# tartarughina/S-BLAS

Hardware: AMD Instinct MI355X
Metric: SpMM GFLOP/s (2*nnz*N/t), CSR x dense N=64, fp64 (higher is better)
Workload: dtype f64; 1 GPU; SpMM method-1 (dense-B column partition), nd24k-like synthetic (M=K=72000, 399 nnz/row, band +-2000, seed 211), nnz=28728000, N=64 columns per GPU, alpha=beta=1, B = srand(211)/rand() as the reference's DenseMatrix, inputs resident in HBM; step = B->row-major staging + row-panel SpMM; rows=72000, cols=72000, nnz=28728000, n_cols_per_gpu=64, parallelism=method1-colblock x1

## Files before the change

include/sblas_hip.h:

```cpp
#ifndef SBLAS_HIP_H
#define SBLAS_HIP_H

#include <stddef.h>
#include <stdint.h>

#ifdef __cplusplus
extern "C" {
#endif

#define SBLAS_OK 0
#define SBLAS_E_INVALID 1
#define SBLAS_E_HIP 2
#define SBLAS_E_WORKSPACE 3
#define SBLAS_E_RCCL 4
#define SBLAS_E_IO 5
#define SBLAS_E_NOGPU 6

int sblas_hip_version(void);
const char *sblas_hip_error_string(int code);
int sblas_hip_device_count(void);

size_t sblas_hip_spmm_csr_f64_i32_workspace(int64_t rows, int64_t cols, int64_t nnz, int64_t n);

int sblas_hip_spmm_csr_f64_i32(int dev, void *stream,
// ... 272 lines not shown
    SBLAS_SPMM_RULE_FOUR_ROWS_WAVES,
    SBLAS_SPMM_RULE_FOUR_ROWS_VOTED,
    SBLAS_SPMM_RULE_MERGE,
    SBLAS_SPMM_RULE_DPP_GROUPS,
    SBLAS_SPMM_RULE_DPP_PAD,
    SBLAS_SPMM_RULE_DPP_LONG,
    SBLAS_SPMM_RULE_NARROW,
    SBLAS_SPMM_RULE_ROWS8,
    SBLAS_SPMM_RULE_INTERLEAVE,
    SBLAS_SPMM_RULE_SKIP,
    SBLAS_SPMM_RULE_SPLIT_GROUPS,
    SBLAS_SPMM_RULE_FIELDS
};
int64_t sblas_spmm_rule_describe(int64_t rows, int64_t cols, int64_t nnz, int64_t ldbt, int64_t n, int64_t ncu,
                                 int caller_staged, const int64_t *plan, int64_t *out, int64_t max_out);

int sblas_host_fill_rand0to1(double *dst, int64_t count, unsigned seed);

int sblas_mm_read_info(const char *path, int32_t *rows, int32_t *cols, int32_t *nnz,
                       int32_t *is_symmetric);
int sblas_mm_read_csr(const char *path, int32_t *rowptr, int32_t *colidx, double *val);

#ifdef __cplusplus
}
#endif
#endif
```

s-blas_amd/csrc/kernels.h:

```cpp
#pragma once
#include <hip/hip_runtime.h>
#include <stdint.h>
#include <vector>
#include "../../include/sblas_hip.h"

namespace sblas {

constexpr int MAX_REPLICAS = 16;
struct ReplicaPtrs {
    double *p[MAX_REPLICAS];
};

enum {
    SPMM_VARIANT_AUTO = 0,
    SPMM_VARIANT_DIRECT_DPP = 1,
    SPMM_VARIANT_DIRECT_ROWS = 2,
    SPMM_VARIANT_LANES = 3,
    SPMM_VARIANT_DIRECT_MERGE = 4,
    SPMM_VARIANT_MFMA = 5,
    SPMM_VARIANT_NO_MFMA = 6,
};
constexpr int SPMM_MIN_PANEL_ROWS = 32;

enum { TAIL_NONFINITE = 0,
// ... 24 lines not shown
__device__ __forceinline__ float c_fma(float a, float b, float c) { return fmaf(a, b, c); }
template <int W, typename T, typename At, typename Keep>
__device__ __forceinline__ void store_rows_c(T *__restrict__ C, int64_t ldc, int64_t row0, int64_t col0, int prows, int nrows,
                                             int ncols, int nthreads, T alpha, T beta, At at, Keep keep)
{
    for (int idx = threadIdx.x; idx < W * prows; idx += nthreads) {
        const int j = idx % W, r = idx / W;
        if (r < nrows && j < ncols && keep(r)) {
            T *dst = C + (row0 + r) * ldc + (col0 + j);
            const T sres = alpha * at(r, j);
            *dst = (beta == T(0)) ? sres : c_fma(beta, *dst, sres);
        }
    }
}

__device__ __forceinline__ int xcd_contiguous_panel(int b, int npanels)
{
    const int xcd = b & 7, idx = b >> 3;
    const int q = npanels >> 3, r = npanels & 7;
    const int base = (xcd < r) ? xcd * (q + 1) : r * (q + 1) + (xcd - r) * q;
    return base + idx;
}

struct Options {
    int spmm_variant = SPMM_VARIANT_AUTO;
    char spmv_variant[16] = {0};
    bool tier16 = true, tier32 = true;
    unsigned long long max_bt_bytes = 0xffffffffull;
    int direct_lds = -1;
    int direct_map = -1;
    int stage_range = -1;
    int direct_merge = 1;
    double rows8_min_avg = 256.0;
    float window_density = 0.42f;
    int panel_rows = 0, panel_groups = 0;
    int lanes_copies = 1;
    size_t mfma_lds_floor = 0;
    bool one_half = false;
    int rowlen_bar = 0;
    int mfma_batch64 = 2;
    int mfma_batch128 = 2;
    int dpp_long = DPP_LONG;
    bool lanes32_one_lane = false;
    int rows_waves = 0;
    bool validate = false;
    float mfma_min_fill = -1.0f;
};
const Options &options();
void options_reload();
int compute_units();
// ... 69 lines not shown
SpmmStep spmm_step(int rows, int cols, int64_t nnz, int64_t ldbt, const PlanView *pv, const SpmmStep &prev = SpmmStep(),
                   bool caller_staged = false);
struct ClassifyArgs {
    int max_row_len;
    float min_density, min_rowlen, mfma_min_fill;
    int merge_probe;
};
ClassifyArgs classify_args(int panel_rows, int64_t ldbt);
int range_parts(int64_t nnz);

enum { TILED_NONE = 0, TILED_WINDOW6 = 1 , TILED_LANES = 2  };
struct SpmmStage2 {
    int tiled = TILED_NONE;
    int g = 0;
    int nh = 0, grid_y = 0;
    int nc = 0, cp = 0, lpe = 0;
    bool mfma = false;
    int mfma_batch = 0;
    size_t mfma_lds_floor = 0;
    bool four_rows = false;
    int rows_waves = 0, voted = 0;
    bool merge = false;
    int dpp = 0;
    size_t dpp_pad = 0;
    int dpp_long = 0;
    int narrow = 0;
    bool rows8 = false;
    int interleave = -1;
    bool skip = false;
    int split_groups = 0;
};
SpmmStage2 spmm_stage2(const SpmmStep &st, int rows, int cols, int64_t nnz, int n);
hipError_t launch_stage(hipStream_t s, const SpmmStep &st, int rows, int64_t cols, int64_t nnz, const int *rowptr,
                        const int *colidx, int64_t n, const double *B, int64_t ldb, double *Bt, bool row_b);
hipError_t launch_spmm_rowpanel(hipStream_t s, const SpmmStep &st, int rows, int cols, int64_t nnz, const int *rowptr,
                                const int *colidx, const double *val, const double *Bt, int n, double alpha, double beta,
                                double *C, int64_t ldc, bool row_c);
hipError_t plan_build(hipStream_t s, const SpmmStep &st, int rows, int cols, int64_t nnz, const int *rowptr, const int *colidx,
                      PlanView *pv, std::vector<int> *cls_out = nullptr);
hipError_t launch_dense_to_rowmajor(hipStream_t s, int64_t cols, int64_t n, const double *B, int64_t ldb,
                                    double *Bt, int64_t ldbt, bool row_b);
hipError_t launch_scale(hipStream_t s, int64_t rows, int64_t n, double beta, double *C, int64_t ldc, bool row_c);
hipError_t validate_csr(hipStream_t s, int64_t rows, int64_t cols, int64_t nnz, const int *rowptr, const int *colidx, int *bad);
hipError_t panel_stats(unsigned long long out[4], bool reset);
hipError_t launch_spmv(hipStream_t s, int rows, int cols, int64_t nnz, const int *rowptr, const int *colidx,
                       const double *val, const double *x, double alpha, double beta, double *y);
int spmv_kind(double avg, int family = -1);
// ... 42 lines not shown
```

s-blas_amd/csrc/kernels.hip:

```cpp
#include <hip/hip_runtime.h>
#include <atomic>
#include <stdint.h>
#include <algorithm>
#include <type_traits>
#include <mutex>
#include <vector>
#include "kernels.h"

namespace sblas {

constexpr int WAVE = 64;

__device__ __forceinline__ int wave_uniform(int v) { return __builtin_amdgcn_readfirstlane(v); }

__device__ __forceinline__ double readlane_f64(double v, int src_lane)
{
    int lo = __double2loint(v), hi = __double2hiint(v);
    lo = __builtin_amdgcn_readlane(lo, src_lane);
    hi = __builtin_amdgcn_readlane(hi, src_lane);
    return __hiloint2double(hi, lo);
}

constexpr int STAGE_K = 32;
template <bool RB>
// ... 207 lines not shown
        for (; k < cnt; ++k) {
            const int c = __builtin_amdgcn_readlane(cj, k);
            const double a = readlane_f64(vj, k);
            acc = fma(a, (Bt + (size_t)((unsigned)c * ld32))[lane_off], acc);
        }
    }
    return acc;
}
#ifndef SBLAS_W2_ROWS
#define SBLAS_W2_ROWS 152
#endif
constexpr int W2_ROWS = SBLAS_W2_ROWS;
constexpr int W2_LROWS = W2_ROWS / 4;
static_assert(W2_ROWS % 8 == 0, "tile rows");
constexpr int W2_TILE = W2_ROWS * 64;
constexpr size_t W2_LDS_BYTES = (2 * (size_t)W2_TILE + 64) * sizeof(double) + 64 * sizeof(int);

constexpr int MFMA_BITMAP_WORDS = 1024;
__device__ __forceinline__ void classify_panel(int p, int rows, int cols, int npanels, int panel_rows,
                                               const int *__restrict__ rowptr, const int *__restrict__ colidx,
                                               ClassifyArgs a, int *__restrict__ tail, int2 *__restrict__ info,
                                               int *__restrict__ cls, int epoch, unsigned *__restrict__ bitmap)
{
    const int max_row_len = a.max_row_len, merge_probe = a.merge_probe;
    const float min_density = a.min_density, min_rowlen = a.min_rowlen, mfma_min_fill = a.mfma_min_fill;
    const int lane = threadIdx.x & 63;
    if (p >= npanels) return;
    int first = 0x7fffffff, last = -1, len = 0, mlen = 0;
    for (int rr = lane; rr < panel_rows; rr += WAVE) {
        const int row = p * panel_rows + rr;
        if (row < rows) {
// ... 426 lines not shown
template <int N> __device__ __forceinline__ void vm_wait6()
{
    static_assert(N == 8 || N == 12, "counts of the sixth-generation tile loop");
    if (N == 12) asm volatile("s_waitcnt vmcnt(12)" ::: "memory");
    else asm volatile("s_waitcnt vmcnt(8)" ::: "memory");
}

template <int G, int NH, bool RC>
__global__ __launch_bounds__(1024) void spmm_window6_kernel(
    int rows, int cols, int npanels, const int *__restrict__ rowptr, const int *__restrict__ colidx,
    const double *__restrict__ val, const double *__restrict__ Bt, int64_t ldbt, int n, double alpha, double beta,
    double *__restrict__ C, int64_t ldc, const int *__restrict__ tail, const int2 *__restrict__ info,
    const int *__restrict__ cls, int panel_rows, int nnz)
{
    constexpr int RW = 4 * G, RMAX = 16 * RW;
    static_assert(G == 2 || G == 3, "two or three groups per wave (the counted vmcnt waits are 4 G)");
    static_assert(NH == 1 || NH == 2, "one or two 64-column halves per workgroup");
    static_assert(64 * (RMAX + 1) <= 2 * W2_TILE, "C tile must fit in the (dead) B tile buffers");
    extern __shared__ __attribute__((aligned(16))) double smem[];
    double *zero_row = smem + 2 * W2_TILE;
    int *sm_i = reinterpret_cast<int *>(smem + 2 * W2_TILE + 64);

    const int panel = xcd_contiguous_panel(blockIdx.x, npanels);
    if (!owns_window(tail, cls, panel)) return;
    const int2 span = info[panel];

    const int tid = threadIdx.x;
    const int lane = tid & 63;
    const int wave = wave_uniform(tid >> 6);
    const int row0 = panel * panel_rows;
    const int col0 = blockIdx.y * (64 * NH);
    const unsigned ld32 = (unsigned)ldbt;
    const int t_lo = span.x / W2_ROWS, t_hi = span.y / W2_ROWS;
    const bool loader = wave >= 12;
    const bool active = !loader && wave * RW < panel_rows;

    if (tid < 64) zero_row[tid] = 0.0;
    if (tid == 0) sm_i[0] = 0;

    double acc[NH][G][4];
#pragma unroll
    for (int h = 0; h < NH; ++h)
#pragma unroll
        for (int g = 0; g < G; ++g)
#pragma unroll
            for (int j = 0; j < 4; ++j) acc[h][g][j] = 0.0;

    const unsigned ldb8 = ld32 * 8u;
    const unsigned piece_off = (unsigned)(col0 + ((lane & 31) << 1)) * 8u;
    const unsigned pair_off = (unsigned)(lane >> 5) * ldb8 + piece_off;
    const char *bt_bytes = reinterpret_cast<const char *>(Bt);
    int dummy = 0;
    auto dma_part = [&](int t, int h, int buf) {
        const int lw = wave - 12;
        const int r0 = t * W2_ROWS + lw * W2_LROWS;
        const unsigned lds0 = (unsigned)wave_uniform((int)((unsigned)(uintptr_t)(smem + buf * W2_TILE) + (unsigned)lw * (unsigned)(W2_LROWS * 512)));
        const unsigned hoff = (unsigned)h * 512u;
        if (r0 + W2_LROWS - 1 <= cols) {
            const char *p = bt_bytes + (size_t)((unsigned)r0 * ldb8) + hoff;
#pragma unroll
            for (int i = 0; i < W2_LROWS / 2; ++i) dma_rows_scalar(lds0 + i * 1024u, pair_off, p + (size_t)(2u * i) * ldb8);
        } else {
#pragma unroll
            for (int i = 0; i < W2_LROWS / 2; ++i) {
                const unsigned brow = (unsigned)min(r0 + 2 * i + (lane >> 5), cols);
                dma_rows_vector(lds0 + i * 1024u, bt_bytes + (size_t)(brow * ldb8 + piece_off + hoff));
            }
        }
    };

    if (loader) dma_part(t_lo, 0, 0);

    const int k = lane & 15, q = lane >> 4;
    const int wrow = min(row0 + wave * RW, rows);
    const int wstart = wave_uniform(rowptr[wrow]);
    const sblas_rsrc_t rc = make_rsrc(colidx + wstart, 4u, (unsigned)(nnz - wstart));
    const sblas_rsrc_t rv = make_rsrc(val + wstart, 8u, (unsigned)(nnz - wstart));
    int cur[G], end[G];
#pragma unroll
    for (int g = 0; g < G; ++g) {
        const int rr = wave * RW + 4 * g + q;
        const int row = row0 + rr;
        cur[g] = end[g] = 0;
        if (rr < panel_rows && row < rows) {
            cur[g] = rowptr[row] - wstart;
            end[g] = rowptr[row + 1] - wstart;
        }
    }
    unsigned long long viol = 0ull;
    int wca[G], wcb[G];
    double wva[G], wvb[G];
    unsigned s_coA[G], s_coB[G];
    double s_gvA[G], s_gvB[G];
    int s_take[G], s_mx[G];
    bool replay[G];
#pragma unroll
    for (int g = 0; g < G; ++g) {
        s_coA[g] = s_coB[g] = 0u;
        s_gvA[g] = s_gvB[g] = 0.0;
        s_take[g] = s_mx[g] = 0;
        replay[g] = false;
    }
#pragma unroll
    for (int g = 0; g < G; ++g) window_issue6(rc, rv, cur[g] + k, wca[g], wva[g], wcb[g], wvb[g]);
    asm volatile("s_waitcnt vmcnt(0)" ::: "memory");
    __syncthreads();
    int step = 0;
    for (int t = t_lo; t <= t_hi; ++t) {
        const int tile_lo = t * W2_ROWS;
        auto half = [&](auto hc) {
            constexpr int h = decltype(hc)::value;
            const int cbuf = step & 1;
            if (loader) {
                if (h + 1 < NH) dma_part(t, h + 1, cbuf ^ 1);
                else if (t < t_hi) dma_part(t + 1, 0, cbuf ^ 1);
            }
            const unsigned tile_base = (unsigned)(uintptr_t)(smem + cbuf * W2_TILE);
            const unsigned lb = tile_base + (unsigned)k * 16u;
            const unsigned zero_rel = (unsigned)(uintptr_t)zero_row - tile_base;
            auto visit = [&](auto gc) {
                constexpr int g = decltype(gc)::value;
                if (h == 0) window_wait6<NH == 1 ? 4 * (G - 1) : 4 * (G - 1 - g)>(wca[g], wva[g], wcb[g], wvb[g]);
                else if (replay[g]) window_wait6<0>(wca[g], wva[g], wcb[g], wvb[g]);
                double &q0 = acc[h][g][0], &q1 = acc[h][g][1], &q2 = acc[h][g][2], &q3 = acc[h][g][3];
                int lc = cur[g];
                bool full = h == 0 || replay[g];
                for (;;) {
                    unsigned coA, coB;
                    double gvA, gvB;
                    int take, mx;
// ... 60 lines not shown
            ++step;
        };
        half(std::integral_constant<int, 0>{});
        if constexpr (NH > 1) half(std::integral_constant<int, 1>{});
    }
#pragma unroll
    for (int g = 0; g < G; ++g) window_wait6<0>(wca[g], wva[g], wcb[g], wvb[g]);
    int bad = viol != 0ull ? 1 : 0;
#pragma unroll
    for (int g = 0; g < G; ++g)
        if (__builtin_amdgcn_ballot_w64(cur[g] < end[g]) != 0ull) bad = 1;
    if (bad && lane == 0) atomicOr(&sm_i[0], 1);
    __syncthreads();
    const bool fell_back = sm_i[0] != 0;
    if (tid == 0 && blockIdx.y == 0) atomicAdd(&g_panel_stats[fell_back ? 2 : 0], 1ull);

    double *ctile = smem;
    const int nrows = min(panel_rows, rows - row0);
#pragma unroll
    for (int h = 0; h < NH; ++h) {
        const int colh = col0 + 64 * h;
        if (fell_back) {
            const unsigned lane_off = (unsigned)(colh + lane);
#pragma unroll
            for (int g = 0; g < G; ++g)
#pragma unroll
                for (int j = 0; j < 4; ++j) {
                    const int rr = wave * RW + 4 * g + j;
                    const int row = row0 + rr;
                    int a = 0, b = 0;
// ... 6 lines not shown
        }
        if (h > 0) __syncthreads();
#pragma unroll
        for (int g = 0; g < G; ++g) {
            if (fell_back) {
#pragma unroll
                for (int j = 0; j < 4; ++j) ctile[lane * (RMAX + 1) + wave * RW + 4 * g + j] = acc[h][g][j];
            } else {
                const int rr = wave * RW + 4 * g + q;
                ctile[(2 * k) * (RMAX + 1) + rr] = acc[h][g][0];
                ctile[(2 * k + 1) * (RMAX + 1) + rr] = acc[h][g][1];
                ctile[(32 + 2 * k) * (RMAX + 1) + rr] = acc[h][g][2];
                ctile[(33 + 2 * k) * (RMAX + 1) + rr] = acc[h][g][3];
            }
        }
        __syncthreads();
        const int ncols = min(64, n - colh);
        if constexpr (RC)
            store_rows_c<64>(C, ldc, row0, colh, panel_rows, nrows, ncols, 1024, alpha, beta,
                             [&](int r, int j) { return ctile[j * (RMAX + 1) + r]; }, [](int) { return true; });
        else
        for (int idx = tid; idx < 64 * panel_rows; idx += 1024) {
            const int r = idx % panel_rows, j = idx / panel_rows;
            if (r < nrows && j < ncols) {
                double *dst = C + (int64_t)(colh + j) * ldc + (row0 + r);
                const double sres = alpha * ctile[j * (RMAX + 1) + r];
                *dst = (beta == 0.0) ? sres : fma(beta, *dst, sres);
            }
        }
    }
}

constexpr int WL_TR = 256;
template <int NC, int CP> struct WlGeom {
    static constexpr int P = NC / 2;
    static constexpr unsigned ROWB = NC * 8;
    static constexpr unsigned ROW = CP * ROWB;
    static constexpr int SHIFT = ROW == 64 ? 6 : ROW == 128 ? 7 : 8;
    static constexpr unsigned TILE = WL_TR * ROW;
    static constexpr size_t LDS_BYTES = 2 * (size_t)TILE + 512 + 64;
    static constexpr int LPR = CP * P;
    static constexpr int RPI = 64 / LPR;
    static_assert(ROW == 64 || ROW == 128 || ROW == 256, "copies x row bytes");
    static_assert(CP * P <= 16, "a lane group has sixteen lanes");
};
// ... 386 lines not shown
    static_assert(GROUPS == 1 || GROUPS == 2 || GROUPS == 4, "lane groups of 64, 32 or 16 lanes");
    constexpr int TILE_COLS = 128 / GROUPS;
    constexpr int GLANES = 64 / GROUPS;
    __shared__ double ctile[TILE_COLS][WIDE_PANEL + 1];
    if (cls != nullptr && nothing_direct(tail, epoch)) return;
    if (GROUPS == 1 && cls != nullptr && (tail[TAIL_MERGE_EPOCH] == epoch || tail[TAIL_ROWS_EPOCH] == epoch)) return;
    const int lane = threadIdx.x & 63;
    const int wave = wave_uniform(threadIdx.x >> 6);
    if (interleave < 0) {
        interleave = 0;
        if (cls != nullptr) {
            const int band = tail[TAIL_BAND];
            interleave = (long long)band * (TILE_COLS * 8) > (16ll << 20);
        }
    }
    const int row0 = (interleave ? (int)blockIdx.x : xcd_contiguous_panel(blockIdx.x, npanels)) * WIDE_PANEL;
    const int col0 = blockIdx.y * TILE_COLS;
    const int row = row0 + wave;
    bool mine = row < rows;
    if (cls && mine) {
        mine = owns_direct(tail, cls, row / info_panel_rows);
        if (mine && lane == 0 && blockIdx.y == 0 && row % info_panel_rows == 0) atomicAdd(&g_panel_stats[1], 1ull);
    }
    if (SKIP && mine) mine = !is_split_row(split_bits, row);
    const int sub = lane & 15;
    const int half = lane / GLANES;
    const unsigned ldb8 = (unsigned)ldbt * 8u;
    const unsigned lb = (unsigned)(col0 * 8) + (unsigned)(lane % GLANES) * 16u;
    const unsigned zero_off = (unsigned)cols * ldb8;
    const char *__restrict__ bt_bytes = reinterpret_cast<const char *>(Bt);

    double acc0 = 0.0, acc1 = 0.0;
    auto sweep = [&](int p0, int p1) { dpp_sweep<GROUPS>(colidx, val, bt_bytes, ldb8, lb, zero_off, lane, sub, half, p0, p1, acc0, acc1); };
    __shared__ int long_wave[WIDE_PANEL];
    __shared__ int n_long;
    if (threadIdx.x == 0) n_long = 0;
    __syncthreads();
    int rp0 = 0, rp1 = 0;
    if (mine) {
        rp0 = wave_uniform(rowptr[row]);
        rp1 = wave_uniform(rowptr[row + 1]);
    }
    const bool is_long = mine && rp1 - rp0 >= long_min;
    if (is_long && lane == 0) long_wave[atomicAdd(&n_long, 1)] = wave;
    if (mine && !is_long) sweep(rp0, rp1);
    if (GROUPS == 4) {
        acc0 += __shfl_xor(acc0, 16, WAVE);
        acc1 += __shfl_xor(acc1, 16, WAVE);
// ... 42 lines not shown
        }
    }
    const int nrows = min(WIDE_PANEL, rows - row0);
    const int ncols = min(TILE_COLS, n - col0);
    if constexpr (RC)
        store_rows_c<TILE_COLS>(C, ldc, row0, col0, WIDE_PANEL, nrows, ncols, WIDE_WAVES * 64, alpha, beta,
                                [&](int r, int j) { return ctile[j][r]; }, [&](int r) { return row_mine[r] != 0; });
    else
    for (int idx = threadIdx.x; idx < TILE_COLS * WIDE_PANEL; idx += WIDE_WAVES * 64) {
        const int r = idx % WIDE_PANEL, j = idx / WIDE_PANEL;
        if (r < nrows && j < ncols && row_mine[r]) {
            double *dst = C + (int64_t)(col0 + j) * ldc + (row0 + r);
            const double sres = alpha * ctile[j][r];
            *dst = (beta == 0.0) ? sres : fma(beta, *dst, sres);
        }
    }
}

constexpr int MR = 3;
constexpr int MERGE_WAVES = 8;
constexpr int MERGE_PANEL = MERGE_WAVES * MR;
template <int NR>
__device__ __forceinline__ void merged_sweeps(int cj, const double (&vj)[NR], int cnt, double (&acc)[NR][2], int sub,
                                              unsigned ldb8, unsigned lb, unsigned zero_off,
                                              const char *__restrict__ bt_bytes)
{
    for (int g0 = 0; g0 < cnt; g0 += 16) {
        const int e = g0 + sub;
        const int src = e << 2;
        const bool on = e < cnt;
// ... 815 lines not shown
    const SpmmStage2 d = spmm_stage2(st, rows, cols, nnz, n);
    const int64_t ldbt = st.ldbt;
    const PlanView *pv = st.pv;
    const Tail t = pv ? tail_at(pv->tail, rows) : tail_of(Bt, cols, ldbt, rows);
    const bool classified = st.verdicts != VERDICTS_NONE;
    const int *cls = classified ? t.cls : nullptr;
    const int info_rows = st.info_rows, np = st.npanels, epoch = st.epoch;
    const unsigned *skip = d.skip ? pv->split_bits : nullptr;
    bool missing = false;
    if (classified && !pv) launch_verdicts(s, st, rows, cols, rowptr, colidx, t, st.verdicts == VERDICTS_SEPARATE);

    if (classified) {
        KernelEvents *kev = kernel_events_slot();
        if (kev) (void)hipEventRecord(kev->a, s);
        if (d.tiled == TILED_WINDOW6) {
            const dim3 wgrid((unsigned)np, (unsigned)d.grid_y);
#define SBLAS_W6_CASE(GG, NH)                                                                                          \
    case GG * 10 + NH:                                                                                                \
        raise_dynamic_lds((const void *)spmm_window6_kernel<GG, NH, RC>, W2_LDS_BYTES);                               \
        hipLaunchKernelGGL((spmm_window6_kernel<GG, NH, RC>), wgrid, dim3(1024), W2_LDS_BYTES, s, rows, cols, np, rowptr,   \
                           colidx, val, Bt, ldbt, n, alpha, beta, C, ldc, t.hdr, t.info, t.cls, info_rows, (int)nnz); \
        break;
            switch (d.g * 10 + d.nh) {
                SBLAS_W6_CASE(2, 1) SBLAS_W6_CASE(2, 2) SBLAS_W6_CASE(3, 1)
            default: missing = true;
            }
#undef SBLAS_W6_CASE
        } else if (d.tiled == TILED_LANES) {
#define SBLAS_LANES_CASE(NC, CP, GG, LPE)                                                                              \
    case ((NC * 10 + CP) * 10 + GG) * 10 + LPE:                                                                       \
        raise_dynamic_lds((const void *)spmm_lanes_kernel<NC, CP, GG, LPE, RC>, WlGeom<NC, CP>::LDS_BYTES);           \
// ... 36 lines not shown
            SBLAS_ROWS_CASE(4) SBLAS_ROWS_CASE(8) SBLAS_ROWS_CASE(16)
        default: missing = true;
        }
#undef SBLAS_ROWS_CASE
    }
    if (d.merge) {
        const int mp = (rows + MERGE_PANEL - 1) / MERGE_PANEL;
        const size_t lds = (size_t)128 * (MERGE_PANEL + 1) * sizeof(double);
        raise_dynamic_lds((const void *)spmm_direct_merge_kernel<RC>, lds);
        hipLaunchKernelGGL(spmm_direct_merge_kernel<RC>, dim3((unsigned)mp, (unsigned)(ldbt / 128)), dim3(MERGE_WAVES * 64), lds,
                           s, rows, cols, mp, rowptr, colidx, val, Bt, ldbt, n, alpha, beta, C, ldc, t.hdr, cls, info_rows,
                           d.interleave, epoch);
    }
    if (d.dpp) {
        const int wide_panels = (rows + WIDE_PANEL - 1) / WIDE_PANEL;
        const dim3 grid((unsigned)wide_panels, d.dpp == 1 ? (unsigned)(ldbt / 128) : 1u);
#define SBLAS_DPP_CASE(GR)                                                                                             \
    case GR:                                                                                                          \
        SBLAS_DIRECT_GO(spmm_direct_dpp_kernel, (GR, RC), grid, dim3(WIDE_WAVES * 64), d.dpp_pad, rows, cols, wide_panels,  \
                        rowptr, colidx, val, Bt, ldbt, n, alpha, beta, C, ldc, t.hdr, cls, info_rows, d.interleave, epoch,   \
                        d.dpp_long);                                                                                  \
        break;
        switch (d.dpp) {
            SBLAS_DPP_CASE(1) SBLAS_DPP_CASE(2) SBLAS_DPP_CASE(4)
        default: missing = true;
        }
#undef SBLAS_DPP_CASE
    }
    if (d.narrow) {
        const unsigned panels = (unsigned)((rows + PANEL_ROWS - 1) / PANEL_ROWS);
#define SBLAS_NARROW_CASE(NC)                                                                                          \
// ... 104 lines not shown
```

s-blas_amd/csrc/spmm_rule.cpp:

```cpp
#include <stdint.h>
#include <stdio.h>
#include <stdlib.h>
#include <string.h>
#include <algorithm>
#include <atomic>
#include <mutex>
#include "../../include/sblas_hip.h"
#include "kernels.h"

namespace sblas {

static Options g_options;
static std::atomic<bool> g_options_loaded{false};
static std::mutex g_options_mu;
static void options_parse(Options &o)
{
    o = Options{};
    const char *e;
    if ((e = getenv("SBLAS_SPMM_VARIANT")) && *e) {
        if (!strcmp(e, "dpp")) o.spmm_variant = SPMM_VARIANT_DIRECT_DPP;
        else if (!strcmp(e, "rows")) o.spmm_variant = SPMM_VARIANT_DIRECT_ROWS;
        else if (!strcmp(e, "lanes")) o.spmm_variant = SPMM_VARIANT_LANES;
        else if (!strcmp(e, "merge")) o.spmm_variant = SPMM_VARIANT_DIRECT_MERGE;
        else if (!strcmp(e, "mfma")) o.spmm_variant = SPMM_VARIANT_MFMA;
// ... 5 lines not shown
    if ((e = getenv("SBLAS_SPMM_MIN_LDBT")) && *e) o.tier16 = o.tier32 = atoi(e) < 64;
    if ((e = getenv("SBLAS_SPMM_MAX_BT_BYTES")) && *e) {
        const unsigned long long v = strtoull(e, nullptr, 10);
        if (v >= 4096 && v < 0xffffffffull) o.max_bt_bytes = v;
    }
    if ((e = getenv("SBLAS_DIRECT_LDS")) && *e) o.direct_lds = atoi(e);
    if ((e = getenv("SBLAS_DIRECT_MERGE")) && *e) o.direct_merge = atoi(e);
    if ((e = getenv("SBLAS_STAGE_RANGE")) && *e) o.stage_range = atoi(e);
    if ((e = getenv("SBLAS_DIRECT_MAP")) && *e) o.direct_map = !strcmp(e, "interleave") ? 1 : !strcmp(e, "contiguous") ? 0 : -1;
    if ((e = getenv("SBLAS_ROWS8_MIN_AVG")) && *e) o.rows8_min_avg = atof(e);
    if ((e = getenv("SBLAS_WINDOW_DENSITY")) && *e) o.window_density = (float)atof(e);
    if ((e = getenv("SBLAS_SPMM_PANEL_ROWS")) && *e) {
        o.panel_rows = atoi(e);
        o.panel_groups = strchr(e, ',') ? atoi(strchr(e, ',') + 1) : 0;
    }
    if ((e = getenv("SBLAS_MFMA_MIN_FILL")) && *e) o.mfma_min_fill = (float)atof(e);
    if ((e = getenv("SBLAS_VALIDATE")) && *e) o.validate = atoi(e) != 0;
    if ((e = getenv("SBLAS_TUNE")) && *e) {
        char buf[96];
        strncpy(buf, e, sizeof buf - 1);
        buf[sizeof buf - 1] = 0;
        for (char *c = buf; *c; ++c)
            if (*c == ':') *c = ',';
        int a = 0, b = 0, c = 0, d = 0;
        sscanf(buf, "%d,%d,%d,%d", &a, &b, &c, &d);
        if (a == 2 || a == 4) o.lanes_copies = a;
        if (a > 0 && a <= 160 * 1024) o.mfma_lds_floor = (size_t)a;
        o.one_half = b == 1;
        if (b > 1) o.rowlen_bar = b;
        if (b == 3 || b == 4) o.mfma_batch64 = b;
// ... 153 lines not shown
        st.npanels = (int)(((int64_t)rows + st.info_rows - 1) / st.info_rows);
    }
    again = classify && range && prev.staging == STAGE_RANGE && prev.verdicts != VERDICTS_NONE && prev.ldbt == ldbt;
    st.verdicts = !classify ? VERDICTS_NONE : again ? VERDICTS_EARLIER : caller_staged ? VERDICTS_SEPARATE : VERDICTS_STAGING;
    return st;
}

SpmmStep spmm_step(int rows, int cols, int64_t nnz, int64_t ldbt, const PlanView *pv, const SpmmStep &prev, bool caller_staged)
{
    bool again = false;
    SpmmStep st = step_rule(rows, cols, nnz, ldbt, pv, prev, caller_staged, 0, again);
    st.epoch = pv ? pv->epoch : again ? prev.epoch : next_epoch();
    return st;
}

SpmmStage2 spmm_stage2(const SpmmStep &st, int rows, int cols, int64_t nnz, int n)
{
    SpmmStage2 d;
    const Options &opt = options();
    const int variant = opt.spmm_variant;
    const int64_t ldbt = st.ldbt;
    const PlanView *pv = st.pv;
    const double avg_row = rows > 0 ? (double)nnz / (double)rows : 0.0;
    const bool classified = st.verdicts != VERDICTS_NONE;
    const bool need_window = !pv || pv->n_window + pv->n_mfma_w > 0;
    const bool need_mfma = !pv || pv->n_mfma_w + pv->n_mfma_d > 0;
    const bool need_direct = !pv || pv->n_direct + pv->n_mfma_d > 0;
    d.g = st.groups;
    d.interleave = opt.direct_map;
    d.dpp_long = opt.dpp_long;
    d.skip = pv && pv->n_split > 0;
    d.split_groups = ldbt >= 128 ? 1 : ldbt == 64 ? 2 : 4;
    d.rows_waves = opt.rows_waves ? opt.rows_waves : avg_row < 8.0 ? 4 : 16;
    if (ldbt >= 64) {
        if (classified) {
            const bool two_halves = ldbt >= 128 && !opt.one_half;
            if (need_window) {
                d.tiled = TILED_WINDOW6;
                d.g = st.groups == 3 ? 3 : 2;
                d.nh = d.g == 2 && two_halves ? 2 : 1;
                d.grid_y = (int)(ldbt / (two_halves ? 128 : 64));
            }
            d.mfma = need_mfma && mfma_min_fill(variant, st.info_rows, ldbt) <= 1.0f;
            d.mfma_batch = ldbt == 64 ? opt.mfma_batch64 : opt.mfma_batch128;
            d.mfma_lds_floor = opt.mfma_lds_floor;
        }
        d.dpp_pad = opt.direct_lds >= 0 ? (size_t)opt.direct_lds : (ldbt == 64 ? 0 : 90000);
        if (!need_direct) {
        } else if (n > 32 && (variant == SPMM_VARIANT_DIRECT_ROWS ||
                              (variant != SPMM_VARIANT_DIRECT_DPP && avg_row < (ldbt == 64 ? 56.0 : 32.0)))) {
            d.four_rows = true;
        } else if (ldbt == 64) {
            d.dpp = n <= 32 ? 4 : 2;
        } else {
            d.merge = pv ? pv->merge : variant == SPMM_VARIANT_DIRECT_MERGE || (classified && opt.direct_merge);
            d.dpp = (pv ? !pv->merge && !pv->four_rows : variant != SPMM_VARIANT_DIRECT_MERGE) ? 1 : 0;
            d.four_rows = pv ? pv->four_rows : classified && variant != SPMM_VARIANT_DIRECT_MERGE;
// ... 43 lines not shown
    if (plan) {
        for (int k = 0; k < SBLAS_SPMM_RULE_PLAN_FIELDS; ++k)
            if (plan[k] < 0) return -1;
        if (plan[SBLAS_SPMM_RULE_PLAN_PANEL_ROWS] < 1 || plan[SBLAS_SPMM_RULE_PLAN_PANEL_ROWS] > INT32_MAX ||
            plan[SBLAS_SPMM_RULE_PLAN_GROUPS] > INT32_MAX || caller_staged)
            return -1;
        pv.n_window = (long)plan[SBLAS_SPMM_RULE_PLAN_N_WINDOW], pv.n_direct = (long)plan[SBLAS_SPMM_RULE_PLAN_N_DIRECT];
        pv.n_mfma_w = (long)plan[SBLAS_SPMM_RULE_PLAN_N_MFMA_W], pv.n_mfma_d = (long)plan[SBLAS_SPMM_RULE_PLAN_N_MFMA_D];
        pv.merge = plan[SBLAS_SPMM_RULE_PLAN_MERGE] != 0, pv.four_rows = plan[SBLAS_SPMM_RULE_PLAN_FOUR_ROWS] != 0;
        pv.n_split = plan[SBLAS_SPMM_RULE_PLAN_N_SPLIT];
        pv.info_rows = (int)plan[SBLAS_SPMM_RULE_PLAN_PANEL_ROWS], pv.groups = (int)plan[SBLAS_SPMM_RULE_PLAN_GROUPS];
    }
    bool again = false;
    const sblas::SpmmStep st = sblas::step_rule((int)rows, (int)cols, nnz, ldbt, plan ? &pv : nullptr, sblas::SpmmStep(),
                                                caller_staged != 0, (int)ncu, again);
    const sblas::SpmmStage2 d = sblas::spmm_stage2(st, (int)rows, (int)cols, nnz, (int)n);
    int64_t f[SBLAS_SPMM_RULE_FIELDS] = {0};
    f[SBLAS_SPMM_RULE_STAGING] = st.staging, f[SBLAS_SPMM_RULE_VERDICTS] = st.verdicts;
    f[SBLAS_SPMM_RULE_PANEL_ROWS] = st.info_rows, f[SBLAS_SPMM_RULE_GROUPS] = st.groups;
    f[SBLAS_SPMM_RULE_PANELS] = st.npanels, f[SBLAS_SPMM_RULE_PLANNABLE] = st.plannable;
    f[SBLAS_SPMM_RULE_TILED] = d.tiled, f[SBLAS_SPMM_RULE_TILED_G] = d.tiled ? d.g : 0;
    f[SBLAS_SPMM_RULE_W6_NH] = d.nh, f[SBLAS_SPMM_RULE_W6_GRID_Y] = d.grid_y;
    f[SBLAS_SPMM_RULE_LANES_NC] = d.nc, f[SBLAS_SPMM_RULE_LANES_CP] = d.cp, f[SBLAS_SPMM_RULE_LANES_LPE] = d.lpe;
    f[SBLAS_SPMM_RULE_MFMA] = d.mfma;
    f[SBLAS_SPMM_RULE_MFMA_BATCH] = d.mfma ? d.mfma_batch : 0;
    f[SBLAS_SPMM_RULE_MFMA_LDS_FLOOR] = d.mfma ? (int64_t)d.mfma_lds_floor : 0;
    f[SBLAS_SPMM_RULE_FOUR_ROWS] = d.four_rows;
    f[SBLAS_SPMM_RULE_FOUR_ROWS_WAVES] = d.four_rows ? d.rows_waves : 0;
    f[SBLAS_SPMM_RULE_FOUR_ROWS_VOTED] = d.voted;
    f[SBLAS_SPMM_RULE_MERGE] = d.merge;
    f[SBLAS_SPMM_RULE_DPP_GROUPS] = d.dpp;
    f[SBLAS_SPMM_RULE_DPP_PAD] = d.dpp ? (int64_t)d.dpp_pad : 0;
    f[SBLAS_SPMM_RULE_DPP_LONG] = d.dpp ? d.dpp_long : 0;
    f[SBLAS_SPMM_RULE_NARROW] = d.narrow, f[SBLAS_SPMM_RULE_ROWS8] = d.rows8;
    f[SBLAS_SPMM_RULE_INTERLEAVE] = d.interleave;
    f[SBLAS_SPMM_RULE_SKIP] = d.skip, f[SBLAS_SPMM_RULE_SPLIT_GROUPS] = d.skip ? d.split_groups : 0;
    for (int64_t k = 0; out && k < SBLAS_SPMM_RULE_FIELDS && k < max_out; ++k) out[k] = f[k];
    return SBLAS_SPMM_RULE_FIELDS;
}
```

s-blas_amd/python/sblas_amd/__init__.py:

```python
import ctypes as C
import os

import numpy as np

_PKG = os.path.dirname(os.path.abspath(__file__))
_ROOT = os.path.normpath(os.path.join(_PKG, "..", ".."))
LIB_PATH = os.environ.get("SBLAS_LIB_PATH") or os.path.join(_ROOT, "lib", "libsblas_hip.so")

EXPORTS = [
    "sblas_hip_version", "sblas_hip_error_string", "sblas_hip_device_count",
    "sblas_hip_spmm_csr_f64_i32_workspace", "sblas_hip_spmm_csr_f64_i32", "sblas_hip_spmm_ldbt",
    "sblas_hip_dense_to_rowmajor_f64", "sblas_hip_spmm_csr_rowmajorB_f64_i32",
    "sblas_hip_debug_spmm_panel_stats", "sblas_hip_debug_reload_env",
    "sblas_hip_debug_spmm_kernel_events", "sblas_hip_debug_spmm_last_kernel_ms", "sblas_hip_spmv_csr_f64_i32", "sblas_hip_axpby_f64",
    "sblas_hip_comm_get", "sblas_hip_comm_release_all", "sblas_hip_allreduce_sum_f64",
    "sblas_hip_merge_rowblocks_f64", "sblas_hip_merge_rowblocks_local_f64",
    "sblas_find_row_of_nnz", "sblas_partition_nnz", "sblas_partition_dense",
    "sblas_mm_read_info", "sblas_mm_read_csr", "sblas_host_fill_rand0to1",
    "sblas_hip_spmm_csr_workspace", "sblas_hip_spmm_csr", "sblas_hip_spmv_csr", "sblas_hip_axpby",
    "sblas_hip_allreduce_sum", "sblas_hip_merge_rowblocks", "sblas_partition_nnz_i64",
    "sblas_hip_debug_validate_csr_i32",
    "sblas_hip_spmm_plan_create", "sblas_hip_spmm_plan_destroy", "sblas_hip_spmm_plan_info", "sblas_hip_spmm_csr_f64_i32_planned",
    "sblas_hip_spmv_plan_create", "sblas_hip_spmv_plan_destroy", "sblas_hip_spmv_plan_info", "sblas_hip_spmv_csr_f64_i32_planned",
    "sblas_spmv_plan_classify",
    "sblas_hip_spmm_csr_ordered", "sblas_hip_spmm_csr_ordered_f64_i32_planned", "sblas_hip_merge_rowblocks_ordered",
    "sblas_hip_spmm_plan_create_split", "sblas_hip_spmm_plan_split_info", "sblas_spmm_split_classify",
    "sblas_spmm_rule_describe",
    "sblas_hip_csr_transpose_workspace", "sblas_hip_csr_transpose_f64_i32", "sblas_hip_gather_f64",
    "sblas_hip_transpose_plan_create", "sblas_hip_transpose_plan_update_values", "sblas_hip_transpose_plan_info",
    "sblas_hip_transpose_plan_csc", "sblas_hip_transpose_plan_destroy", "sblas_hip_spmv_csr_t_f64_i32_planned",
    "sblas_hip_spmm_csr_t_f64_i32_planned",
    "sblas_hip_coo_to_csr_workspace", "sblas_hip_coo_to_csr_f64_i32", "sblas_hip_coo_plan_create", "sblas_hip_coo_plan_info",
    "sblas_hip_coo_plan_csr", "sblas_hip_coo_plan_assemble", "sblas_hip_coo_plan_destroy",
    "sblas_hip_sddmm_csr_workspace", "sblas_hip_sddmm_csr_f64_i32",
    "sblas_hip_csr_softmax_workspace", "sblas_hip_csr_softmax_f64_i32", "sblas_hip_csr_softmax_backward_f64_i32",
    "sblas_hip_csr_attention_workspace", "sblas_hip_csr_attention_f64_i32", "sblas_hip_csr_attention_backward_f64_i32",
    "sblas_hip_spgemm_limits", "sblas_hip_spgemm_classify", "sblas_hip_spgemm_group_width", "sblas_hip_spgemm_check_nnz",
    "sblas_hip_spgemm_plan_create", "sblas_hip_spgemm_plan_info", "sblas_hip_spgemm_plan_csr", "sblas_hip_spgemm_plan_numeric",
    "sblas_hip_spgemm_plan_destroy",
    "sblas_hip_sptrsv_limits", "sblas_sptrsv_levels", "sblas_sptrsv_schedule",
    "sblas_hip_sptrsv_plan_create", "sblas_hip_sptrsv_plan_info", "sblas_hip_sptrsv_plan_order", "sblas_hip_sptrsv_plan_destroy",
    "sblas_hip_sptrsv_f64_i32_planned", "sblas_hip_sptrsm_f64_i32_planned",
# ... 26 lines not shown
    L.sblas_hip_spmm_csr_f64_i32_workspace.argtypes = [i64, i64, i64, i64]
    L.sblas_hip_spmm_csr_f64_i32.restype = C.c_int
    L.sblas_hip_spmm_csr_f64_i32.argtypes = [C.c_int, vp, i64, i64, i64, vp, vp, vp, vp, i64, i64, f64, f64, vp, i64, vp, sz]
    L.sblas_hip_debug_validate_csr_i32.restype = C.c_int
    L.sblas_hip_debug_validate_csr_i32.argtypes = [C.c_int, vp, i64, i64, i64, vp, vp]
    L.sblas_hip_spmm_plan_create.restype = C.c_int
    L.sblas_hip_spmm_plan_create.argtypes = [C.c_int, vp, i64, i64, i64, vp, vp, i64, C.POINTER(vp)]
    L.sblas_hip_spmm_plan_create_split.restype = C.c_int
    L.sblas_hip_spmm_plan_create_split.argtypes = [C.c_int, vp, i64, i64, i64, vp, vp, i64, i64, i64, C.POINTER(vp)]
    L.sblas_hip_spmm_plan_split_info.restype = C.c_int
    L.sblas_hip_spmm_plan_split_info.argtypes = [vp, C.POINTER(i64)]
    L.sblas_spmm_split_classify.restype = i64
    L.sblas_spmm_split_classify.argtypes = [vp, i64, i64, i64, i64, vp, i64, vp, i64]
    L.sblas_spmm_rule_describe.restype = i64
    L.sblas_spmm_rule_describe.argtypes = [i64, i64, i64, i64, i64, i64, C.c_int, vp, vp, i64]
    L.sblas_hip_spmm_plan_destroy.restype = C.c_int
    L.sblas_hip_spmm_plan_destroy.argtypes = [vp]
    L.sblas_hip_spmm_plan_info.restype = C.c_int
    L.sblas_hip_spmm_plan_info.argtypes = [vp, C.POINTER(i64)]
    L.sblas_hip_spmm_csr_f64_i32_planned.restype = C.c_int
    L.sblas_hip_spmm_csr_f64_i32_planned.argtypes = [vp, C.c_int, vp, i64, i64, i64, vp, vp, vp, vp, i64, i64, f64, f64, vp, i64, vp, sz]
    L.sblas_hip_spmv_plan_create.restype = C.c_int
    L.sblas_hip_spmv_plan_create.argtypes = [C.c_int, vp, i64, i64, i64, vp, vp, C.POINTER(vp)]
    L.sblas_hip_spmv_plan_destroy.restype = C.c_int
    L.sblas_hip_spmv_plan_destroy.argtypes = [vp]
    L.sblas_hip_spmv_plan_info.restype = C.c_int
    L.sblas_hip_spmv_plan_info.argtypes = [vp, C.POINTER(i64)]
    L.sblas_hip_spmv_csr_f64_i32_planned.restype = C.c_int
    L.sblas_hip_spmv_csr_f64_i32_planned.argtypes = [vp, C.c_int, vp, i64, i64, i64, vp, vp, vp, vp, f64, f64, vp]
    L.sblas_spmv_plan_classify.restype = i64
# ... 1495 lines not shown
```

Measured before the change: 15530 GFLOP/s.

## Make window6 and direct-DPP SpMM kernels persistent with next-panel prefetch

The window6 row-panel kernel becomes persistent: its grid is capped near the CU count and each workgroup walks panels in rounds. While it finishes the current panel it prefetches the next panel's row pointers, spans and first B tile into LDS, so the next panel's startup overlaps the current epilogue. The direct-DPP kernel likewise loops over wide panels with a grid capped at four times the CU count. The aim is to cut launch and tail imbalance and hide per-panel startup latency, at the cost of more complex synchronisation, more LDS for the row-pointer records, and the risk of load imbalance from static round-robin assignment.

```diff
diff --git a/include/sblas_hip.h b/include/sblas_hip.h
--- a/include/sblas_hip.h
+++ b/include/sblas_hip.h
@@ -310,6 +310,7 @@
 };
 int64_t sblas_spmm_rule_describe(int64_t rows, int64_t cols, int64_t nnz, int64_t ldbt, int64_t n, int64_t ncu,
                                  int caller_staged, const int64_t *plan, int64_t *out, int64_t max_out);
+int64_t sblas_spmm_walk_describe(int64_t npanels, int64_t grid, int64_t ncu, int64_t *out, int64_t max_out);
 
 int sblas_host_fill_rand0to1(double *dst, int64_t count, unsigned seed);
 
diff --git a/s-blas_amd/csrc/kernels.h b/s-blas_amd/csrc/kernels.h
--- a/s-blas_amd/csrc/kernels.h
+++ b/s-blas_amd/csrc/kernels.h
@@ -62,12 +62,17 @@
     }
 }
 
-__device__ __forceinline__ int xcd_contiguous_panel(int b, int npanels)
+__host__ __device__ __forceinline__ int xcd_contiguous_panel(int b, int npanels)
 {
     const int xcd = b & 7, idx = b >> 3;
     const int q = npanels >> 3, r = npanels & 7;
     const int base = (xcd < r) ? xcd * (q + 1) : r * (q + 1) + (xcd - r) * q;
     return base + idx;
+}
+__host__ __device__ __forceinline__ int walk_panel(int b, int r, int grid, int npanels)
+{
+    const long long v = (long long)b + (long long)r * grid;
+    return v < npanels ? xcd_contiguous_panel((int)v, npanels) : -1;
 }
 
 struct Options {
@@ -82,6 +87,7 @@
     double rows8_min_avg = 256.0;
     float window_density = 0.42f;
     int panel_rows = 0, panel_groups = 0;
+    int w6_grid = 0;
     int lanes_copies = 1;
     size_t mfma_lds_floor = 0;
     bool one_half = false;
@@ -181,6 +187,7 @@
     int tiled = TILED_NONE;
     int g = 0;
     int nh = 0, grid_y = 0;
+    int grid_x = 0;
     int nc = 0, cp = 0, lpe = 0;
     bool mfma = false;
     int mfma_batch = 0;
@@ -194,10 +201,12 @@
     int narrow = 0;
     bool rows8 = false;
     int interleave = -1;
+    int direct_cap = 0;
     bool skip = false;
     int split_groups = 0;
 };
-SpmmStage2 spmm_stage2(const SpmmStep &st, int rows, int cols, int64_t nnz, int n);
+SpmmStage2 spmm_stage2(const SpmmStep &st, int rows, int cols, int64_t nnz, int n, int ncu = 0);
+int w6_grid_x(int npanels, int ncu);
 hipError_t launch_stage(hipStream_t s, const SpmmStep &st, int rows, int64_t cols, int64_t nnz, const int *rowptr,
                         const int *colidx, int64_t n, const double *B, int64_t ldb, double *Bt, bool row_b);
 hipError_t launch_spmm_rowpanel(hipStream_t s, const SpmmStep &st, int rows, int cols, int64_t nnz, const int *rowptr,
diff --git a/s-blas_amd/csrc/kernels.hip b/s-blas_amd/csrc/kernels.hip
--- a/s-blas_amd/csrc/kernels.hip
+++ b/s-blas_amd/csrc/kernels.hip
@@ -245,7 +245,10 @@
 constexpr int W2_LROWS = W2_ROWS / 4;
 static_assert(W2_ROWS % 8 == 0, "tile rows");
 constexpr int W2_TILE = W2_ROWS * 64;
-constexpr size_t W2_LDS_BYTES = (2 * (size_t)W2_TILE + 64) * sizeof(double) + 64 * sizeof(int);
+constexpr int W6_SM_INTS = 256, W6_REC = 8, W6_REC_RP = 12;
+static_assert(W6_REC_RP + 48 * W6_GMAX + 1 <= W6_SM_INTS, "row pointers of the tallest panel");
+constexpr size_t W2_LDS_BYTES = (2 * (size_t)W2_TILE + 64) * sizeof(double) + W6_SM_INTS * sizeof(int);
+static_assert(W2_LDS_BYTES <= 160 * 1024, "LDS of a CU");
 
 constexpr int MFMA_BITMAP_WORDS = 1024;
 __device__ __forceinline__ void classify_panel(int p, int rows, int cols, int npanels, int panel_rows,
@@ -702,37 +705,38 @@
     const int *__restrict__ cls, int panel_rows, int nnz)
 {
     constexpr int RW = 4 * G, RMAX = 16 * RW;
+    constexpr int PARK_BYTES = 64 * (RMAX + 1) * 8, TILE_BYTES = W2_TILE * 8;
     static_assert(G == 2 || G == 3, "two or three groups per wave (the counted vmcnt waits are 4 G)");
     static_assert(NH == 1 || NH == 2, "one or two 64-column halves per workgroup");
     static_assert(64 * (RMAX + 1) <= 2 * W2_TILE, "C tile must fit in the (dead) B tile buffers");
     extern __shared__ __attribute__((aligned(16))) double smem[];
     double *zero_row = smem + 2 * W2_TILE;
     int *sm_i = reinterpret_cast<int *>(smem + 2 * W2_TILE + 64);
-
-    const int panel = xcd_contiguous_panel(blockIdx.x, npanels);
-    if (!owns_window(tail, cls, panel)) return;
+    int *rec = sm_i + W6_REC, *rec_rp = sm_i + W6_REC_RP;
+
+    const int grid = gridDim.x, wg = blockIdx.x;
+    int round = 0, panel;
+    for (;; ++round) {
+        panel = walk_panel(wg, round, grid, npanels);
+        if (panel < 0 || owns_window(tail, cls, panel)) break;
+    }
+    if (panel < 0) return;
     const int2 span = info[panel];
 
     const int tid = threadIdx.x;
     const int lane = tid & 63;
     const int wave = wave_uniform(tid >> 6);
-    const int row0 = panel * panel_rows;
+    int row0 = panel * panel_rows;
     const int col0 = blockIdx.y * (64 * NH);
     const unsigned ld32 = (unsigned)ldbt;
-    const int t_lo = span.x / W2_ROWS, t_hi = span.y / W2_ROWS;
+    int t_lo = span.x / W2_ROWS, t_hi = span.y / W2_ROWS;
     const bool loader = wave >= 12;
     const bool active = !loader && wave * RW < panel_rows;
 
     if (tid < 64) zero_row[tid] = 0.0;
-    if (tid == 0) sm_i[0] = 0;
+    if (tid == 0) sm_i[0] = 0, rec[0] = -1;
 
     double acc[NH][G][4];
-#pragma unroll
-    for (int h = 0; h < NH; ++h)
-#pragma unroll
-        for (int g = 0; g < G; ++g)
-#pragma unroll
-            for (int j = 0; j < 4; ++j) acc[h][g][j] = 0.0;
 
     const unsigned ldb8 = ld32 * 8u;
     const unsigned piece_off = (unsigned)(col0 + ((lane & 31) << 1)) * 8u;
@@ -757,31 +761,45 @@
         }
     };
 
-    if (loader) dma_part(t_lo, 0, 0);
+    if (loader) dma_part(t_lo, 0, 1);
 
     const int k = lane & 15, q = lane >> 4;
-    const int wrow = min(row0 + wave * RW, rows);
-    const int wstart = wave_uniform(rowptr[wrow]);
-    const sblas_rsrc_t rc = make_rsrc(colidx + wstart, 4u, (unsigned)(nnz - wstart));
-    const sblas_rsrc_t rv = make_rsrc(val + wstart, 8u, (unsigned)(nnz - wstart));
+    sblas_rsrc_t rc, rv;
     int cur[G], end[G];
-#pragma unroll
-    for (int g = 0; g < G; ++g) {
-        const int rr = wave * RW + 4 * g + q;
-        const int row = row0 + rr;
-        cur[g] = end[g] = 0;
-        if (rr < panel_rows && row < rows) {
-            cur[g] = rowptr[row] - wstart;
-            end[g] = rowptr[row + 1] - wstart;
-        }
-    }
-    unsigned long long viol = 0ull;
+    auto row_state = [&](int prow0, auto rp) {
+        const int wstart = wave_uniform(rp(min(wave, 12) * RW));
+        rc = make_rsrc(colidx + wstart, 4u, (unsigned)(nnz - wstart));
+        rv = make_rsrc(val + wstart, 8u, (unsigned)(nnz - wstart));
+#pragma unroll
+        for (int g = 0; g < G; ++g) {
+            const int rr = wave * RW + 4 * g + q;
+            cur[g] = end[g] = 0;
+            if (rr < panel_rows && prow0 + rr < rows) {
+                cur[g] = rp(rr) - wstart;
+                end[g] = rp(rr + 1) - wstart;
+            }
+        }
+    };
+    row_state(row0, [&](int i) { return rowptr[min(row0 + i, rows)]; });
+    unsigned long long viol;
     int wca[G], wcb[G];
     double wva[G], wvb[G];
     unsigned s_coA[G], s_coB[G];
     double s_gvA[G], s_gvB[G];
     int s_take[G], s_mx[G];
     bool replay[G];
+    if (!loader) {
+#pragma unroll
+        for (int g = 0; g < G; ++g) window_issue6(rc, rv, cur[g] + k, wca[g], wva[g], wcb[g], wvb[g]);
+    }
+  for (;;) {
+#pragma unroll
+    for (int h = 0; h < NH; ++h)
+#pragma unroll
+        for (int g = 0; g < G; ++g)
+#pragma unroll
+            for (int j = 0; j < 4; ++j) acc[h][g][j] = 0.0;
+    viol = 0ull;
 #pragma unroll
     for (int g = 0; g < G; ++g) {
         s_coA[g] = s_coB[g] = 0u;
@@ -789,11 +807,13 @@
         s_take[g] = s_mx[g] = 0;
         replay[g] = false;
     }
-#pragma unroll
-    for (int g = 0; g < G; ++g) window_issue6(rc, rv, cur[g] + k, wca[g], wva[g], wcb[g], wvb[g]);
     asm volatile("s_waitcnt vmcnt(0)" ::: "memory");
+    if (!loader) {
+#pragma unroll
+        for (int g = 0; g < G; ++g) window_wait6<0>(wca[g], wva[g], wcb[g], wvb[g]);
+    }
     __syncthreads();
-    int step = 0;
+    int step = 1;
     for (int t = t_lo; t <= t_hi; ++t) {
         const int tile_lo = t * W2_ROWS;
         auto half = [&](auto hc) {
@@ -802,6 +822,20 @@
             if (loader) {
                 if (h + 1 < NH) dma_part(t, h + 1, cbuf ^ 1);
                 else if (t < t_hi) dma_part(t + 1, 0, cbuf ^ 1);
+                if (h == 0 && t == t_lo && wave == 12) {
+                    int nr = round + 1, np;
+                    for (;; ++nr) {
+                        np = walk_panel(wg, nr, grid, npanels);
+                        if (np < 0 || owns_window(tail, cls, np)) break;
+                    }
+                    if (np >= 0) {
+                        const int2 sp = info[np];
+                        const int nrow0 = np * panel_rows;
+                        for (int i = lane; i <= 12 * RW; i += 64) rec_rp[i] = rowptr[min(nrow0 + i, rows)];
+                        if (lane == 0) rec[1] = nr, rec[2] = sp.x, rec[3] = sp.y;
+                    }
+                    if (lane == 0) rec[0] = np;
+                }
             }
             const unsigned tile_base = (unsigned)(uintptr_t)(smem + cbuf * W2_TILE);
             const unsigned lb = tile_base + (unsigned)k * 16u;
@@ -892,6 +926,15 @@
     __syncthreads();
     const bool fell_back = sm_i[0] != 0;
     if (tid == 0 && blockIdx.y == 0) atomicAdd(&g_panel_stats[fell_back ? 2 : 0], 1ull);
+    const int nextp = wave_uniform(rec[0]);
+    int nround = 0, nrow0 = 0, n_tlo = 0, n_thi = 0;
+    if (nextp >= 0) {
+        nround = wave_uniform(rec[1]);
+        nrow0 = nextp * panel_rows;
+        n_tlo = wave_uniform(rec[2]) / W2_ROWS, n_thi = wave_uniform(rec[3]) / W2_ROWS;
+    }
+    const bool dma_early = TILE_BYTES + (wave - 12) * (W2_LROWS * 512) >= PARK_BYTES;
+    if (loader && nextp >= 0 && dma_early) dma_part(n_tlo, 0, 1);
 
     double *ctile = smem;
     const int nrows = min(panel_rows, rows - row0);
@@ -928,7 +971,17 @@
                 ctile[(33 + 2 * k) * (RMAX + 1) + rr] = acc[h][g][3];
             }
         }
+        if (h == NH - 1) {
+            if (nextp >= 0) {
+                row_state(nrow0, [&](int i) { return rec_rp[i]; });
+                if (!loader) {
+#pragma unroll
+                    for (int g = 0; g < G; ++g) window_issue6(rc, rv, cur[g] + k, wca[g], wva[g], wcb[g], wvb[g]);
+                }
+            }
+        }
         __syncthreads();
+        if (h == NH - 1 && tid == 0) sm_i[0] = 0, rec[0] = -1;
         const int ncols = min(64, n - colh);
         if constexpr (RC)
             store_rows_c<64>(C, ldc, row0, colh, panel_rows, nrows, ncols, 1024, alpha, beta,
@@ -943,6 +996,13 @@
             }
         }
     }
+    if (nextp < 0) break;
+    if constexpr (PARK_BYTES > TILE_BYTES) {
+        __syncthreads();
+        if (loader && !dma_early) dma_part(n_tlo, 0, 1);
+    }
+    panel = nextp, round = nround, row0 = nrow0, t_lo = n_tlo, t_hi = n_thi;
+  }
 }
 
 constexpr int WL_TR = 256;
@@ -1359,15 +1419,7 @@
             interleave = (long long)band * (TILE_COLS * 8) > (16ll << 20);
         }
     }
-    const int row0 = (interleave ? (int)blockIdx.x : xcd_contiguous_panel(blockIdx.x, npanels)) * WIDE_PANEL;
     const int col0 = blockIdx.y * TILE_COLS;
-    const int row = row0 + wave;
-    bool mine = row < rows;
-    if (cls && mine) {
-        mine = owns_direct(tail, cls, row / info_panel_rows);
-        if (mine && lane == 0 && blockIdx.y == 0 && row % info_panel_rows == 0) atomicAdd(&g_panel_stats[1], 1ull);
-    }
-    if (SKIP && mine) mine = !is_split_row(split_bits, row);
     const int sub = lane & 15;
     const int half = lane / GLANES;
     const unsigned ldb8 = (unsigned)ldbt * 8u;
@@ -1375,8 +1427,26 @@
     const unsigned zero_off = (unsigned)cols * ldb8;
     const char *__restrict__ bt_bytes = reinterpret_cast<const char *>(Bt);
 
-    double acc0 = 0.0, acc1 = 0.0;
+    double acc0, acc1;
     auto sweep = [&](int p0, int p1) { dpp_sweep<GROUPS>(colidx, val, bt_bytes, ldb8, lb, zero_off, lane, sub, half, p0, p1, acc0, acc1); };
+    bool used_lds = false;
+    for (int vb = blockIdx.x; vb < npanels; vb += gridDim.x) {
+    const int row0 = (interleave ? vb : xcd_contiguous_panel(vb, npanels)) * WIDE_PANEL;
+    const int row = row0 + wave;
+    bool mine = row < rows;
+    if (cls) {
+        const int p_lo = row0 / info_panel_rows, p_hi = min(row0 + WIDE_PANEL - 1, rows - 1) / info_panel_rows;
+        const bool own_lo = owns_direct(tail, cls, p_lo), own_hi = p_hi == p_lo ? own_lo : owns_direct(tail, cls, p_hi);
+        if (!own_lo && !own_hi) continue;
+        if (mine) {
+            mine = row / info_panel_rows == p_lo ? own_lo : own_hi;
+            if (mine && lane == 0 && blockIdx.y == 0 && row % info_panel_rows == 0) atomicAdd(&g_panel_stats[1], 1ull);
+        }
+    }
+    if (SKIP && mine) mine = !is_split_row(split_bits, row);
+    if (used_lds) __syncthreads();
+    used_lds = true;
+    acc0 = acc1 = 0.0;
     __shared__ int long_wave[WIDE_PANEL];
     __shared__ int n_long;
     if (threadIdx.x == 0) n_long = 0;
@@ -1449,6 +1519,7 @@
             const double sres = alpha * ctile[j][r];
             *dst = (beta == 0.0) ? sres : fma(beta, *dst, sres);
         }
+    }
     }
 }
 
@@ -2294,7 +2365,7 @@
         KernelEvents *kev = kernel_events_slot();
         if (kev) (void)hipEventRecord(kev->a, s);
         if (d.tiled == TILED_WINDOW6) {
-            const dim3 wgrid((unsigned)np, (unsigned)d.grid_y);
+            const dim3 wgrid((unsigned)d.grid_x, (unsigned)d.grid_y);
 #define SBLAS_W6_CASE(GG, NH)                                                                                          \
     case GG * 10 + NH:                                                                                                \
         raise_dynamic_lds((const void *)spmm_window6_kernel<GG, NH, RC>, W2_LDS_BYTES);                               \
@@ -2361,7 +2432,8 @@
     }
     if (d.dpp) {
         const int wide_panels = (rows + WIDE_PANEL - 1) / WIDE_PANEL;
-        const dim3 grid((unsigned)wide_panels, d.dpp == 1 ? (unsigned)(ldbt / 128) : 1u);
+        const dim3 grid((unsigned)(d.direct_cap > 0 ? std::min(wide_panels, d.direct_cap) : wide_panels),
+                        d.dpp == 1 ? (unsigned)(ldbt / 128) : 1u);
 #define SBLAS_DPP_CASE(GR)                                                                                             \
     case GR:                                                                                                          \
         SBLAS_DIRECT_GO(spmm_direct_dpp_kernel, (GR, RC), grid, dim3(WIDE_WAVES * 64), d.dpp_pad, rows, cols, wide_panels,  \
diff --git a/s-blas_amd/csrc/spmm_rule.cpp b/s-blas_amd/csrc/spmm_rule.cpp
--- a/s-blas_amd/csrc/spmm_rule.cpp
+++ b/s-blas_amd/csrc/spmm_rule.cpp
@@ -43,6 +43,7 @@
         o.panel_rows = atoi(e);
         o.panel_groups = strchr(e, ',') ? atoi(strchr(e, ',') + 1) : 0;
     }
+    if ((e = getenv("SBLAS_W6_GRID")) && *e) o.w6_grid = atoi(e) > 0 ? atoi(e) : 0;
     if ((e = getenv("SBLAS_MFMA_MIN_FILL")) && *e) o.mfma_min_fill = (float)atof(e);
     if ((e = getenv("SBLAS_VALIDATE")) && *e) o.validate = atoi(e) != 0;
     if ((e = getenv("SBLAS_TUNE")) && *e) {
@@ -226,10 +227,19 @@
     return st;
 }
 
-SpmmStage2 spmm_stage2(const SpmmStep &st, int rows, int cols, int64_t nnz, int n)
+int w6_grid_x(int npanels, int ncu)
+{
+    int g = std::min(npanels, std::max(ncu, 1));
+    const int cap = options().w6_grid;
+    if (cap > 0) g = std::min(g, cap);
+    return std::max(g, 1);
+}
+
+SpmmStage2 spmm_stage2(const SpmmStep &st, int rows, int cols, int64_t nnz, int n, int ncu)
 {
     SpmmStage2 d;
     const Options &opt = options();
+    if (ncu <= 0 && st.verdicts != VERDICTS_NONE && st.ldbt >= 64) ncu = compute_units();
     const int variant = opt.spmm_variant;
     const int64_t ldbt = st.ldbt;
     const PlanView *pv = st.pv;
@@ -252,7 +262,9 @@
                 d.g = st.groups == 3 ? 3 : 2;
                 d.nh = d.g == 2 && two_halves ? 2 : 1;
                 d.grid_y = (int)(ldbt / (two_halves ? 128 : 64));
+                d.grid_x = w6_grid_x(st.npanels, ncu);
             }
+            d.direct_cap = 4 * ncu;
             d.mfma = need_mfma && mfma_min_fill(variant, st.info_rows, ldbt) <= 1.0f;
             d.mfma_batch = ldbt == 64 ? opt.mfma_batch64 : opt.mfma_batch128;
             d.mfma_lds_floor = opt.mfma_lds_floor;
@@ -326,7 +338,7 @@
     bool again = false;
     const sblas::SpmmStep st = sblas::step_rule((int)rows, (int)cols, nnz, ldbt, plan ? &pv : nullptr, sblas::SpmmStep(),
                                                 caller_staged != 0, (int)ncu, again);
-    const sblas::SpmmStage2 d = sblas::spmm_stage2(st, (int)rows, (int)cols, nnz, (int)n);
+    const sblas::SpmmStage2 d = sblas::spmm_stage2(st, (int)rows, (int)cols, nnz, (int)n, (int)ncu);
     int64_t f[SBLAS_SPMM_RULE_FIELDS] = {0};
     f[SBLAS_SPMM_RULE_STAGING] = st.staging, f[SBLAS_SPMM_RULE_VERDICTS] = st.verdicts;
     f[SBLAS_SPMM_RULE_PANEL_ROWS] = st.info_rows, f[SBLAS_SPMM_RULE_GROUPS] = st.groups;
@@ -350,3 +362,14 @@
     for (int64_t k = 0; out && k < SBLAS_SPMM_RULE_FIELDS && k < max_out; ++k) out[k] = f[k];
     return SBLAS_SPMM_RULE_FIELDS;
 }
+
+extern "C" int64_t sblas_spmm_walk_describe(int64_t npanels, int64_t grid, int64_t ncu, int64_t *out, int64_t max_out)
+{
+    if (npanels < 0 || npanels > INT32_MAX || grid > INT32_MAX || ncu < 1 || ncu > INT32_MAX || (out && max_out < 0)) return -1;
+    const int g = grid >= 1 ? (int)grid : sblas::w6_grid_x((int)npanels, (int)ncu);
+    const int64_t rounds = (npanels + g - 1) / g;
+    for (int64_t r = 0; out && r < rounds; ++r)
+        for (int b = 0; b < g; ++b)
+            if (r * g + b < max_out) out[r * g + b] = sblas::walk_panel(b, (int)r, g, (int)npanels);
+    return rounds * g;
+}
diff --git a/s-blas_amd/python/sblas_amd/__init__.py b/s-blas_amd/python/sblas_amd/__init__.py
--- a/s-blas_amd/python/sblas_amd/__init__.py
+++ b/s-blas_amd/python/sblas_amd/__init__.py
@@ -25,7 +25,7 @@
     "sblas_spmv_plan_classify",
     "sblas_hip_spmm_csr_ordered", "sblas_hip_spmm_csr_ordered_f64_i32_planned", "sblas_hip_merge_rowblocks_ordered",
     "sblas_hip_spmm_plan_create_split", "sblas_hip_spmm_plan_split_info", "sblas_spmm_split_classify",
-    "sblas_spmm_rule_describe",
+    "sblas_spmm_rule_describe", "sblas_spmm_walk_describe",
     "sblas_hip_csr_transpose_workspace", "sblas_hip_csr_transpose_f64_i32", "sblas_hip_gather_f64",
     "sblas_hip_transpose_plan_create", "sblas_hip_transpose_plan_update_values", "sblas_hip_transpose_plan_info",
     "sblas_hip_transpose_plan_csc", "sblas_hip_transpose_plan_destroy", "sblas_hip_spmv_csr_t_f64_i32_planned",
@@ -82,6 +82,8 @@
     L.sblas_spmm_split_classify.argtypes = [vp, i64, i64, i64, i64, vp, i64, vp, i64]
     L.sblas_spmm_rule_describe.restype = i64
     L.sblas_spmm_rule_describe.argtypes = [i64, i64, i64, i64, i64, i64, C.c_int, vp, vp, i64]
+    L.sblas_spmm_walk_describe.restype = i64
+    L.sblas_spmm_walk_describe.argtypes = [i64, i64, i64, vp, i64]
     L.sblas_hip_spmm_plan_destroy.restype = C.c_int
     L.sblas_hip_spmm_plan_destroy.argtypes = [vp]
     L.sblas_hip_spmm_plan_info.restype = C.c_int
```

Result: slower. 14780 GFLOP/s (-4.8%).
